# nghiant03/spine-vision

Measured on AMD Instinct MI355X. Metric: images/sec training, ConvNeXt-base 512x512 loc, bs32, at 1/2/4/8 MI355X, higher is better.
Workload: dtype bf16; 1 GPU; CoordinateRegressor(convnext_base) localization train step fwd+bwd+allreduce+clip+AdamW; image_size=512, batch_per_gpu=32, global_batch=32, parallelism=dp1, hip_graph=False

## Files before the change

### include/sv_kernels.h

```cpp
#ifndef SV_KERNELS_H
#define SV_KERNELS_H

#include <stdint.h>

#ifdef __cplusplus
extern "C" {
#endif

typedef struct ihipStream_t* sv_stream_t;

typedef enum { SV_F32 = 0, SV_BF16 = 1 } sv_dtype;

typedef enum {
  SV_OK = 0,
  SV_ERR_INVALID_ARG = 1,
  SV_ERR_UNSUPPORTED = 2,
  SV_ERR_LAUNCH = 3
} sv_status;

int sv_version(void);
const char* sv_last_error_string(void);
const char* sv_build_target(void);

typedef struct sv_ctx sv_ctx;
// ... 372 lines not shown
                   void* out, int32_t out_dtype, int64_t rows, int32_t C, int32_t* ctl, float* ws, sv_stream_t stream);
int sv_bn_bwd_apply_fold(int32_t mode, const void* dout, int32_t dout_dtype, const uint8_t* pool_idx, int32_t pool_H,
                         int32_t pool_W, const void* y, int32_t y_dtype, const float* mean, const float* rstd,
                         const float* gamma, const float* beta, const void* y2, int32_t y2_dtype, const float* mean2,
                         const float* rstd2, const float* gamma2, const float* part, const float* part2,
                         int32_t nparts, void* dx, void* dx2, int32_t dx_dtype, float* dgamma, float* dbeta,
                         float* dgamma2, float* dbeta2, int32_t batch_stats, int64_t rows, int32_t C, int32_t* ctl,
                         float* ws, sv_stream_t stream);
int sv_relu_mask(const void* dout, int32_t dout_dtype, const void* act, int32_t act_dtype, float* g, int64_t n,
                 sv_stream_t stream);
int sv_maxpool3s2_fwd(const void* x, int32_t x_dtype, void* y, uint8_t* idx, int32_t B, int32_t H, int32_t W,
                      int32_t C, sv_stream_t stream);
int sv_maxpool3s2_bwd(const void* dout, int32_t dout_dtype, const uint8_t* idx, void* dx, int32_t dx_dtype,
                      int32_t B, int32_t H, int32_t W, int32_t C, sv_stream_t stream);
int sv_avgpool_fwd(const void* x, int32_t x_dtype, float* feat, int32_t B, int32_t HW, int32_t C,
                   sv_stream_t stream);
int sv_avgpool_bwd(const float* dfeat, void* dx, int32_t dx_dtype, int32_t B, int32_t HW, int32_t C,
                   sv_stream_t stream);

#define SV_HEAD_CE 0
#define SV_HEAD_BCE 1
typedef struct {
  int32_t kind;
  int32_t offset;
  int32_t ncls;
  float weight;
  float label_smoothing;
  const void* target;
  int32_t target_dtype;
} sv_head_task;
int sv_head_loss(const float* logits, int32_t B, int32_t K, const sv_head_task* tasks, int32_t ntasks, float* loss,
                 float* dlogits, sv_stream_t stream);

#ifdef __cplusplus
}
#endif
#endif
```

### spine-vision_amd/kernels.py

```python

from __future__ import annotations

import ctypes
import os

import numpy as np
import torch

from . import native as nv
from .native import SV_BF16, SV_F32, call, dt, ptr, value

EPS_LN = 1e-6


class GemmProbe:

    def __init__(self, key: tuple, name: str = "") -> None:
        self.key = key
        self.name = name
        self.events: list[tuple[torch.cuda.Event, torch.cuda.Event]] = []
        self.flops = 0.0
        self.bytes = 0.0
        self.launches = 0
        self.shares: list[float] = []
# ... 1958 lines not shown
         ptr(rstd), ptr(gamma), ptr(beta), C, ptr(part))
    if (bn_fold_ok(rows, C, P) and rows * C < 2 ** 31
            and _bn_small_args_ok(dpool4d, y2d, mean, rstd, gamma, beta)):
        return _bn_bwd_apply_fold(nv.SV_BN_SMALL_RELU, dpool4d, y2d, mean, rstd, gamma, part, P, idx=idx, H=H, W=W,
                                  beta=beta, dgamma=dgamma, dbeta=dbeta, dx_dtype=dx_dtype, batch_stats=batch_stats,
                                  out=out)
    sums = _bn_bwd_sums(P, C, batch_stats, (part, dgamma, dbeta), sums=sums)
    dx = (torch.empty(rows, C, device=y2d.device, dtype=dx_dtype) if out is None
          else _conv_buf(out, (rows, C), dx_dtype, y2d.device, "bn_relu_bwd_pooled: out"))
    call("sv_bn_relu_bwd_apply_pool", ptr(dpool4d), dt(dpool4d), ptr(idx), B, H, W, ptr(y2d), dt(y2d), ptr(mean),
         ptr(rstd), ptr(gamma), ptr(beta), ptr(sums), ptr(dx), dt(dx), C)
    return dx


def head_loss(logits: torch.Tensor, specs: list) -> tuple:
    _check(logits.dtype == torch.float32 and logits.dim() == 2 and logits.is_contiguous(), "head_loss: logits")
    B, Kc = logits.shape
    cover = 0
    tasks = []
    for kind, off, n, w, sm, t in specs:
        if kind == nv.SV_HEAD_CE:
            _check(t.dtype == torch.int64 and t.is_contiguous() and t.numel() == B, "head_loss: CE target int64 [B]")
        else:
            _check(t.dtype in (torch.float32, torch.bfloat16) and t.is_contiguous() and t.numel() == B * n,
                   "head_loss: BCE target f32 / bf16 [B][ncls]")
        tasks.append(nv.HeadTask(kind, off, n, float(w), float(sm), ptr(t), dt(t) if kind == nv.SV_HEAD_BCE else 0))
        cover += n
    loss = torch.empty((), device=logits.device, dtype=torch.float32)
    dl = (torch.empty_like if cover == Kc else torch.zeros_like)(logits)
    call("sv_head_loss", ptr(logits), B, Kc, (nv.HeadTask * len(tasks))(*tasks), len(tasks), ptr(loss), ptr(dl))
    return loss, dl


def maxpool_fwd(x4d: torch.Tensor, *, out: tuple | None = None):
    B, H, W, C = x4d.shape
    _check(x4d.is_contiguous() and C % 4 == 0, "maxpool_fwd: need contiguous NHWC, C % 4 == 0")
    OH, OW = conv_out_hw(H, W, 3, 2, 1)
    if out is None:
        y = torch.empty(B, OH, OW, C, device=x4d.device, dtype=x4d.dtype)
        idx = torch.empty(B, OH, OW, C, device=x4d.device, dtype=torch.uint8)
    else:
        y = _conv_buf(out[0], (B, OH, OW, C), x4d.dtype, x4d.device, "maxpool_fwd: out")
        idx = _conv_buf(out[1], (B, OH, OW, C), torch.uint8, x4d.device, "maxpool_fwd: out")
    call("sv_maxpool3s2_fwd", ptr(x4d), dt(x4d), ptr(y), ptr(idx), B, H, W, C)
    return y, idx


def maxpool_bwd(dout4d: torch.Tensor, idx: torch.Tensor, H: int, W: int, dx_dtype=torch.float32, *,
                out: torch.Tensor | None = None) -> torch.Tensor:
    B, OH, OW, C = dout4d.shape
    _check(dout4d.is_contiguous() and idx.shape == dout4d.shape and (OH, OW) == conv_out_hw(H, W, 3, 2, 1),
           "maxpool_bwd: shape mismatch")
    dx = (torch.empty(B, H, W, C, device=dout4d.device, dtype=dx_dtype) if out is None
          else _conv_buf(out, (B, H, W, C), dx_dtype, dout4d.device, "maxpool_bwd: out"))
    call("sv_maxpool3s2_bwd", ptr(dout4d), dt(dout4d), ptr(idx), ptr(dx), dt(dx), B, H, W, C)
    return dx


def avgpool_fwd(x4d: torch.Tensor, *, out: torch.Tensor | None = None) -> torch.Tensor:
    B, H, W, C = x4d.shape
    _check(x4d.is_contiguous() and C % 4 == 0, "avgpool_fwd: need contiguous NHWC, C % 4 == 0")
    feat = (torch.empty(B, C, device=x4d.device, dtype=torch.float32) if out is None
            else _conv_buf(out, (B, C), torch.float32, x4d.device, "avgpool_fwd: out"))
    call("sv_avgpool_fwd", ptr(x4d), dt(x4d), ptr(feat), B, H * W, C)
    return feat

# ... 11 lines not shown
```

### spine-vision_amd/native.py

```python

from __future__ import annotations

import ctypes
import os
import re
import threading

import torch

_HERE = os.path.dirname(os.path.abspath(__file__))
LIB_PATH = os.environ.get("SV_LIB_PATH") or os.path.join(_HERE, "libsv_kernels.so")
HEADER = os.path.join(os.path.dirname(_HERE), "include", "sv_kernels.h")

SV_F32, SV_BF16 = 0, 1
SV_IMG_F32_NCHW, SV_IMG_U8_GRAY, SV_IMG_U8_HWC = 0, 1, 2
SV_BN_SMALL_MASK, SV_BN_SMALL_RELU, SV_BN_SMALL_DUAL = 0, 1, 2
SV_HEAD_CE, SV_HEAD_BCE = 0, 1
SV_BN_FOLD_CTL_INTS, SV_BN_FOLD_WS_FLOATS = 256, 2 * 2 * 2048 + 2 * 64 * 16 * 64
(SV_EPI_STORE, SV_EPI_BIAS_GELU2, SV_EPI_BIAS_GAMMA_RES, SV_EPI_GELU_GRAD, SV_EPI_SLAB, SV_EPI_BIAS_GELU_DUAL,
 SV_EPI_MUL_AUX, SV_EPI_BIAS_GELU, SV_EPI_STORE_STATS, SV_EPI_STORE_BN_BWD, SV_EPI_LN_BWD) = range(11)

_p = ctypes.c_void_p
_i32 = ctypes.c_int32
_i64 = ctypes.c_int64
_f32 = ctypes.c_float


class BnRef(ctypes.Structure):
    _fields_ = [("mean", _p), ("rstd", _p), ("gamma", _p), ("beta", _p)]


class GemmPolicy(ctypes.Structure):
    _fields_ = [("impl", _i32), ("grid_cap", _i32), ("wg_per_cu", _i32), ("priority", _i32)]

    def __repr__(self) -> str:
        return (f"GemmPolicy(impl={self.impl}, grid_cap={self.grid_cap}, wg_per_cu={self.wg_per_cu}, "
                f"priority={self.priority})")


class CtxInfo(ctypes.Structure):
    _fields_ = [("device", _i32), ("compute_units", _i32), ("lds_bytes_per_wg", _i32), ("xcds", _i32),
                ("lds_raised_kernels", _i32), ("refs", _i32), ("arch", ctypes.c_char * 32)]


def policy(impl: int = 0, grid_cap: int = 0, wg_per_cu: int = 0, priority: int = 0) -> GemmPolicy:
    return GemmPolicy(int(impl), int(grid_cap or 0), int(wg_per_cu), int(priority))


class GemmDesc(ctypes.Structure):
    _fields_ = [
# ... 149 lines not shown
    "sv_rowscale_add": [_p, _p, _p, _p, _i64, _i64, _i32, _i32, _p],
    "sv_rowscale_cast_bf16": [_p, _p, _p, _i64, _i64, _i32, _i32, _p],
    "sv_patchify16": [_p, _i32, _p, _p, _p, _i32, _i32, _i32, _i32, _i64, _i32, _p],
    "sv_vit_tokens": [_p, _p, _p, _p, _i32, _i32, _i32, _i32, _i32, _p],
    "sv_image_to_nhwc": [_p, _p, _i32, _i32, _i32, _i32, _i32, _i32, _p],
    "sv_image_u8_hwc_to_nhwc": [_p, _p, _p, _p, _i32, _i32, _i32, _i32, _i32, _p],
    "sv_bn_nparts": [_i64, _i32],
    "sv_bn_stats": [_p, _i32, _i64, _i32, _p, _p],
    "sv_bn_stats_finish": [_p, _i32, _p, _i32, _i64, _i32, _f32, _f32, _p, _p, _p, _p, _p, _p, _p, _p],
    "sv_bn_eval_params": [_p, _p, _f32, _p, _p, _i32, _p],
    "sv_bn_act_fwd": [_p, _i32, _p, _p, _p, _p, _p, _i32, _p, _p, _p, _p, _i32, _p, _i32, _i64, _i32, _p],
    "sv_bn_bwd_stats": [_p, _i32, _p, _i32, _p, _i32, _p, _p, _i64, _i32, _p, _p],
    "sv_bn_bwd_stats_mask": [_p, _i32, _p, _i32, _p, _i32, _p, _p, _i64, _i32, _p, _p],
    "sv_bn_bwd_finish": [_p, _i32, _i32, _p, _p, _p, _p, _p, _p],
    "sv_bn_bwd_stats_mask_dual": [_p, _i32, _p, _i32, _p, _i32, _p, _p, _p, _i32, _p, _p, _i64, _i32, _p, _p, _p],
    "sv_bn_bwd_apply_dual": [_p, _i32, _p, _i32, _p, _p, _p, _p, _p, _i32, _p, _p, _p, _p, _p, _p, _i32, _i64, _i32,
                             _p],
    "sv_bn_relu_bwd_stats": [_p, _i32, _p, _i32, _p, _p, _p, _p, _i64, _i32, _p, _p],
    "sv_bn_relu_bwd_apply": [_p, _i32, _p, _i32, _p, _p, _p, _p, _p, _p, _i32, _i64, _i32, _p],
    "sv_bn_relu_bwd_stats_pool": [_p, _i32, _p, _i32, _i32, _i32, _p, _i32, _p, _p, _p, _p, _i32, _p, _p],
    "sv_bn_relu_bwd_apply_pool": [_p, _i32, _p, _i32, _i32, _i32, _p, _i32, _p, _p, _p, _p, _p, _p, _i32, _i32, _p],
    "sv_bn_bwd_apply": [_p, _i32, _p, _i32, _p, _i32, _p, _p, _p, _p, _p, _i32, _p, _i64, _i32, _p],
    "sv_bn_small_ok": [_i64, _i32],
    "sv_bn_bwd_small": [_i32, _p, _i32, _p, _i32, _p, _i32, _p, _p, _p, _p, _p, _i32, _p, _p, _p, _p, _i32, _p, _p,
                        _i32, _p, _p, _p, _p, _i32, _i64, _i32, _p],
    "sv_bn_act_small": [_p, _i32, _p, _i32, _f32, _f32, _p, _p, _p, _p, _p, _p, _p, _p, _i32, _p, _i32, _f32, _f32,
                        _p, _p, _p, _p, _p, _p, _p, _i32, _p, _i32, _i64, _i32, _p],
    "sv_bn_fold_ok": [_i64, _i32, _i32],
    "sv_bn_act_fold": [_p, _i32, _p, _i32, _f32, _f32, _p, _p, _p, _p, _p, _p, _p, _p, _i32, _p, _i32, _f32, _f32,
                       _p, _p, _p, _p, _p, _p, _p, _i32, _p, _i32, _i64, _i32, _p, _p, _p],
    "sv_bn_bwd_apply_fold": [_i32, _p, _i32, _p, _i32, _i32, _p, _i32, _p, _p, _p, _p, _p, _i32, _p, _p, _p, _p, _p,
                             _i32, _p, _p, _i32, _p, _p, _p, _p, _i32, _i64, _i32, _p, _p, _p],
    "sv_head_loss": [_p, _i32, _i32, _p, _i32, _p, _p, _p],
    "sv_relu_mask": [_p, _i32, _p, _i32, _p, _i64, _p],
    "sv_maxpool3s2_fwd": [_p, _i32, _p, _p, _i32, _i32, _i32, _i32, _p],
    "sv_maxpool3s2_bwd": [_p, _i32, _p, _p, _i32, _i32, _i32, _i32, _i32, _p],
    "sv_avgpool_fwd": [_p, _i32, _p, _i32, _i32, _i32, _p],
    "sv_avgpool_bwd": [_p, _p, _i32, _i32, _i32, _i32, _p],
}
_RESTYPES = {"sv_last_error_string": ctypes.c_char_p, "sv_build_target": ctypes.c_char_p,
             "sv_conv_bwd_weight_work_floats": ctypes.c_int64, "sv_gconv_bwd_weight_work_floats": ctypes.c_int64}
_VALUE_FNS = {n for n in _SIGS if n.endswith(("_nparts", "_ws"))} | {"sv_version", "sv_bn_fold_ok", "sv_dwconv7_ln_fused_ok", "sv_conv_bwd_weight_work_floats",
                                                                     "sv_stream_create_cu_reserved", "sv_bn_small_ok",
                                                                     "sv_gconv_bwd_weight_work_floats"}

_NOSTREAM_FNS = {"sv_ctx_create", "sv_ctx_destroy", "sv_ctx_get_info"}

_lib = None
_lock = threading.Lock()


def header_symbols(path: str = HEADER) -> list[str]:
    text = open(path).read()
    text = re.sub(r"/\*.*?\*/", "", text, flags=re.S)
    return sorted(set(re.findall(r"\b(sv_[a-z0-9_]+)\s*\(", text)))


def lib() -> ctypes.CDLL:
    global _lib
    if _lib is not None:
        return _lib
    with _lock:
        if _lib is not None:
            return _lib
        if not os.path.exists(LIB_PATH):
            raise RuntimeError(
                f"spine_vision_amd: native kernel library not found at {LIB_PATH}; "
                "run `python __graft_entry__.py` (hipcc --offload-arch=gfx950) first"
            )
        L = ctypes.CDLL(LIB_PATH)
        missing = [s for s in header_symbols() if not hasattr(L, s)]
        if missing:
            raise RuntimeError(f"spine_vision_amd: {LIB_PATH} lacks symbols {missing}")
        for name, args in _SIGS.items():
            fn = getattr(L, name)
            fn.argtypes = args
# ... 161 lines not shown
```

### spine-vision_amd/training/engine.py

```python

from __future__ import annotations

import os
from collections import deque
from typing import Any, Callable

import torch
import torch.distributed as dist

from .. import kernels as K
from .comm import BufferSync, GradBucketer, broadcast_parameters
from .flat import FlatArena
from .optim import FlatAdamW


class InflightLimiter:

    def __init__(self, max_inflight: int | None = None) -> None:
        if max_inflight is None:
            max_inflight = int(os.environ.get("SV_MAX_INFLIGHT", "2"))
        self.max_inflight = int(max_inflight)
        self._events: deque = deque()

    def step_done(self) -> None:
# ... 214 lines not shown
            static = _clone(inputs)
            torch.cuda.synchronize(self.device)
            graph = torch.cuda.CUDAGraph()
            with torch.cuda.graph(graph):
                self.optimizer.zero_grad()
                loss = fn(self.model, *static)
                loss.backward()
                scale = None
                if self.grad_clip:
                    nc = K.grad_clip_coef(self.arena.grad_flat, self.grad_clip)
                    self.last_grad_norm = nc[0:1]
                    scale = nc[1:2]
                self.optimizer.step_graph(ranges, hyper, grad_scale=scale)
                loss = loss.detach()
            ent = self._graphs[key] = _Graphed(static, graph, loss, hyper, ranges)
        slot = ent.replays % len(ent.ring)
        if ent.ring_events[slot] is not None:
            ent.ring_events[slot].synchronize()
        buf = ent.ring[slot]
        buf.copy_(torch.tensor(vals, dtype=torch.float32))
        ent.hyper.copy_(buf, non_blocking=True)
        ev = torch.cuda.Event()
        ev.record()
        ent.ring_events[slot] = ev
        ent.replays += 1
        _copy_into(ent.static_inputs, inputs)
        ent.graph.replay()
        out = ent.loss.clone()
        if self.limiter is not None:
            self.limiter.step_done()
        return out

    def step_localization(self, image: torch.Tensor, coords: torch.Tensor, mask: torch.Tensor) -> torch.Tensor:
        return self.step_graphed(lambda m, x, c, k: m.get_loss(m(x), c, mask=k), (image, coords, mask))

    def step_classification(self, image: torch.Tensor, targets: dict[str, Any]) -> torch.Tensor:
        return self.step_graphed(lambda m, x, t: m.get_loss(m(x), t), (image, targets))
```

### spine-vision_amd/training/models/generic.py

```python

from __future__ import annotations

import os
from typing import Any, Literal

import numpy as np
import torch
import torch.nn as nn
import torch.nn.functional as F

from ...core.tasks import (
    TaskConfig,
    compute_predictions_for_tasks,
    compute_probabilities_for_tasks,
    create_loss_functions,
    get_strategy,
    get_tasks,
)
from ...native import SV_HEAD_BCE, SV_HEAD_CE
from .backbone import BackboneFactory


class BaseModel(nn.Module):

    @property
    def name(self) -> str:
        raise NotImplementedError

    def predict(self, x: torch.Tensor, **kwargs: Any):
        self.eval()
        with torch.no_grad():
            return self.forward(x, **kwargs)

    def count_parameters(self) -> int:
        return sum(p.numel() for p in self.parameters() if p.requires_grad)

    def freeze_backbone(self) -> None:
        for p in self.backbone.parameters():
            p.requires_grad = False

    def unfreeze_backbone(self) -> None:
        for p in self.backbone.parameters():
            p.requires_grad = True

    def get_features(self, x: torch.Tensor) -> torch.Tensor:
        return self.backbone(x)


_FUSED_HEADS = os.environ.get("SV_FUSED_HEADS", "1") != "0"
_FUSED_LOSS = os.environ.get("SV_FUSED_LOSS", "1") != "0"


class _HeadOutputs(dict):

    logits: torch.Tensor


class _FusedHeadLoss(torch.autograd.Function):

    @staticmethod
    def forward(ctx, logits, specs, *targets):
        from ...kernels import head_loss

        loss, dl = head_loss(logits.detach(), [sp + (t,) for sp, t in zip(specs, targets)])
        ctx.save_for_backward(dl)
        return loss

    @staticmethod
    def backward(ctx, g):
        (dl,) = ctx.saved_tensors
        return (dl * g, None) + (None,) * (len(ctx.needs_input_grad) - 2)


class Classifier(BaseModel):
    def __init__(self, backbone: str = "resnet50", tasks: list[TaskConfig] | None = None, pretrained: bool = True,
                 dropout: float = 0.3, freeze_backbone: bool = False, precision: str | None = None,
                 img_size=None) -> None:
        super().__init__()
        self._backbone_name = backbone
        self._tasks = tasks if tasks is not None else get_tasks()
        self._task_names = [t.name for t in self._tasks]
        self.backbone, self._feature_dim = BackboneFactory.create(backbone, pretrained, precision=precision,
                                                                       img_size=img_size)
        self.dropout = nn.Dropout(dropout)
        self.heads = nn.ModuleDict({t.name: nn.Linear(self._feature_dim, t.num_classes) for t in self._tasks})
        self._loss_functions, self._loss_weights = create_loss_functions(self._tasks)
        if freeze_backbone:
            self.freeze_backbone()

    @property
    def name(self) -> str:
        return f"Classifier-{self._backbone_name}"

    @property
    def task_names(self) -> list[str]:
        return self._task_names

    @property
    def tasks(self) -> list[TaskConfig]:
        return self._tasks

    @property
    def feature_dim(self) -> int:
        return self._feature_dim
# ... 81 lines not shown
        self._num_outputs, self._num_levels = num_outputs, num_levels
        self._loss_type = loss_type
        self.backbone, self._feature_dim = BackboneFactory.create(backbone, pretrained, precision=precision,
                                                                       img_size=img_size)
        self.head = nn.Sequential(
            nn.LayerNorm(self._feature_dim),
            nn.Dropout(dropout),
            nn.Linear(self._feature_dim, 256),
            nn.GELU(),
            nn.Dropout(dropout / 2),
            nn.Linear(256, num_levels * num_outputs),
            nn.Sigmoid(),
        )
        if loss_type not in ("mse", "smooth_l1", "huber"):
            raise ValueError(f"Unknown loss type: {loss_type}")
        if freeze_backbone:
            self.freeze_backbone()

    @property
    def name(self) -> str:
        return f"Regressor-{self._backbone_name}"

    @property
    def feature_dim(self) -> int:
        return self._feature_dim

    @property
    def num_levels(self) -> int:
        return self._num_levels

    def forward(self, x: torch.Tensor, **kwargs: Any) -> torch.Tensor:
        return self.head(self.backbone(x)).view(-1, self._num_levels, self._num_outputs)

    def _elementwise(self, pred: torch.Tensor, target: torch.Tensor) -> torch.Tensor:
        if self._loss_type == "mse":
            return F.mse_loss(pred, target, reduction="none")
        if self._loss_type == "smooth_l1":
            return F.smooth_l1_loss(pred, target, reduction="none", beta=1.0)
        return F.huber_loss(pred, target, reduction="none", delta=0.1)

    def get_loss(self, predictions: torch.Tensor, targets: torch.Tensor, mask: torch.Tensor | None = None,
                 **kwargs: Any) -> torch.Tensor:
        elem = self._elementwise(predictions, targets)
        if mask is None:
            return elem.mean()
        m = (mask != 0).to(elem.dtype).unsqueeze(-1).expand_as(elem)
        return (elem * m).sum() / m.sum().clamp(min=1.0)
```

### spine-vision_amd/training/trainers/localization.py

```python

from __future__ import annotations

from pathlib import Path
from typing import Any, Literal

import numpy as np
import torch

from ..datasets.localization import (
    IDX_TO_LEVEL,
    NUM_LEVELS,
    LocalizationCollator,
    LocalizationDataset,
)
from ..metrics import LocalizationMetrics
from ..models.generic import CoordinateRegressor
from .base import BaseTrainer, TrainingConfig, TrainingResult, logger


class LocalizationConfig(TrainingConfig):
    task: str = "localization"
    backbone: str = "convnext_base"
    pretrained: bool = True
    freeze_backbone_epochs: int = 0
# ... 19 lines not shown
            model = CoordinateRegressor(backbone=config.backbone, num_outputs=2, pretrained=config.pretrained,
                                        dropout=config.dropout, freeze_backbone=config.freeze_backbone_epochs > 0,
                                        num_levels=config.num_levels, loss_type=config.loss_type,
                                        precision=config.effective_precision, img_size=tuple(config.image_size))
        if train_dataset is None:
            train_dataset = LocalizationDataset(Path(config.data_path), split="train", val_ratio=config.val_split,
                                                series_types=config.series_types, sources=config.sources,
                                                image_size=config.image_size, augment=config.augment,
                                                device_transform=config.device_transform,
                                                augment_coords=config.augment_coords)
        if val_dataset is None:
            val_dataset = LocalizationDataset(Path(config.data_path), split="val", val_ratio=config.val_split,
                                              series_types=config.series_types, sources=config.sources,
                                              image_size=config.image_size, augment=False,
                                              device_transform=config.device_transform)
        super().__init__(config, model, train_dataset, val_dataset)
        self.metrics = LocalizationMetrics(pck_thresholds=config.pck_thresholds,
                                           level_names=list(IDX_TO_LEVEL.values()))
        self._backbone_unfrozen = config.freeze_backbone_epochs == 0

    def _collate_fn(self):
        return LocalizationCollator()

    def _unpack_batch(self, batch: dict[str, Any]):
        return batch["image"], batch["coords"]

    def _train_step(self, batch: dict[str, Any]) -> torch.Tensor:
        from ... import kernels as K

        dev = self.device
        image = K.device_images(batch, dev)
        coords = batch["coords"].to(dev, non_blocking=True)
        mask = batch["mask"].to(dev, non_blocking=True)
        return self._optimize(lambda: self.model.get_loss(self.model(image), coords, mask=mask))

    def _validate_epoch(self) -> tuple[float, dict[str, float]]:
        from ... import kernels as K

        self.model.eval()
        total, n = 0.0, 0
        P, T, Mk = [], [], []
        dev = self.device
        with torch.no_grad():
            for batch in self.val_loader:
                coords, mask = (batch[k].to(dev) for k in ("coords", "mask"))
                image = K.device_images(batch, dev) if "resize" in batch else batch["image"].to(dev)
                pred = self.model(image)
                total += float(self.model.get_loss(pred, coords, mask=mask))
                n += 1
                P.append(self._gather(pred).cpu())
                T.append(self._gather(coords).cpu())
                Mk.append(self._gather(mask).cpu())
        if not P:
            return 0.0, {}
        fp, ft, fl = self._flatten_with_mask(torch.cat(P), torch.cat(T), torch.cat(Mk))
        return total / n, self.metrics.compute(fp, ft, fl)

    @staticmethod
    def _flatten_with_mask(predictions, targets, masks):
        sel = masks.numpy() > 0
        lv = np.broadcast_to(np.arange(predictions.shape[1]), sel.shape)
        return predictions.numpy()[sel], targets.numpy()[sel], lv[sel]

    def _compute_metrics(self, predictions, targets) -> dict[str, float]:
        return self.metrics.compute(predictions.numpy(), targets.numpy())

# ... 37 lines not shown
```

Before: 1144 images/sec.

## Fuse localization head LN-MLP-sigmoid-loss into native forward and backward kernels

Adds a native HIP localization head that runs LayerNorm, dropout, FC1, GELU, dropout, FC2, sigmoid and the masked regression loss in two forward kernels, and computes all head gradients in two backward kernels. The trainer and engine call it through a new loss_from_batch path guarded by shape checks. The goal is to replace the many small PyTorch ops and launches in the head and loss with a few fused launches. The head is tiny next to the ConvNeXt-base backbone, so the effect on the whole step is likely small. Dropout masks now come from native_dropout on a cached ones tensor, which changes how randomness is generated.

```diff
diff --git a/include/sv_kernels.h b/include/sv_kernels.h
--- a/include/sv_kernels.h
+++ b/include/sv_kernels.h
@@ -428,6 +428,21 @@
 int sv_head_loss(const float* logits, int32_t B, int32_t K, const sv_head_task* tasks, int32_t ntasks, float* loss,
                  float* dlogits, sv_stream_t stream);
 
+#define SV_LOC_MSE 0
+#define SV_LOC_SMOOTH_L1 1
+#define SV_LOC_HUBER 2
+int sv_loc_head_ok(int32_t F, int32_t H, int32_t O, int32_t L);
+int sv_loc_head_fwd(const float* feat, const float* lnw, const float* lnb, float eps, const float* W1,
+                    const float* b1, const float* W2, const float* b2, const uint8_t* m1, float s1,
+                    const uint8_t* m2, float s2, const float* target, const float* mask, int32_t kind, int32_t B,
+                    int32_t F, int32_t H, int32_t O, int32_t L, float* mean, float* rstd, float* h, float* pred,
+                    float* loss, float* dz, float* dh, float* a, sv_stream_t stream);
+int sv_loc_head_bwd(const float* gout, const float* feat, const float* lnw, const float* lnb, const float* W1,
+                    const uint8_t* m1, float s1, const float* mean, const float* rstd, const float* a,
+                    const float* dz, const float* dh, int32_t B, int32_t F, int32_t H, int32_t O, float* dW1,
+                    float* db1, float* dW2, float* db2, float* dlnw, float* dlnb, float* dxn, float* dfeat,
+                    sv_stream_t stream);
+
 #ifdef __cplusplus
 }
 #endif
diff --git a/spine-vision_amd/csrc/lochead.hip b/spine-vision_amd/csrc/lochead.hip
--- /dev/null
+++ b/spine-vision_amd/csrc/lochead.hip
@@ -0,0 +1,426 @@
+#include <math.h>
+
+#include "common.h"
+
+namespace sv {
+namespace lochead {
+
+constexpr int kH = 256;
+constexpr int kMaxF = 2048;
+constexpr int kKF = kMaxF / 64;
+constexpr int kMaxO = 32;
+constexpr int kRows1 = 4;
+constexpr int kJT = 64;
+constexpr int kRT = 8;
+constexpr int kBC = 32;
+
+__device__ __forceinline__ void gelu_exact(float x, float& g, float& dg) {
+  const float cdf = 0.5f * (1.0f + erff(x * 0.70710678118654752f));
+  const float pdf = 0.3989422804014327f * expf(-0.5f * x * x);
+  g = x * cdf;
+  dg = fmaf(x, pdf, cdf);
+}
+
+__device__ __forceinline__ float ln_drop(float x, float mean, float rstd, float w, float b, float keep) {
+  return fmaf((x - mean) * rstd, w, b) * keep;
+}
+
+__global__ void __launch_bounds__(256) fwd1_kernel(const float* __restrict__ feat, const float* __restrict__ lnw,
+                                                   const float* __restrict__ lnb, float eps,
+                                                   const float* __restrict__ W1, const float* __restrict__ b1,
+                                                   const uint8_t* __restrict__ m1, float s1, int B, int F,
+                                                   float* __restrict__ mean_o, float* __restrict__ rstd_o,
+                                                   float* __restrict__ h) {
+  __shared__ float xs[kRows1][kMaxF];
+  const int lane = threadIdx.x & 63, w = threadIdx.x >> 6;
+  const int KF = F >> 6;
+  const int b = blockIdx.y * kRows1 + w;
+  const int j = blockIdx.x * kRows1 + w;
+  const float* wr = W1 + (size_t)j * F;
+  float wj[kKF];
+#pragma unroll
+  for (int k = 0; k < kKF; ++k) wj[k] = k < KF ? wr[lane + 64 * k] : 0.f;
+  const float bj = b1[j];
+  if (b < B) {
+    const float* xr = feat + (size_t)b * F;
+    float x[kKF], lw[kKF], lb[kKF], keep[kKF];
+#pragma unroll
+    for (int k = 0; k < kKF; ++k) {
+      const int f = lane + 64 * k;
+      x[k] = k < KF ? xr[f] : 0.f;
+      lw[k] = k < KF ? lnw[f] : 0.f;
+      lb[k] = k < KF ? lnb[f] : 0.f;
+      keep[k] = (k < KF && m1) ? (m1[(size_t)b * F + f] ? s1 : 0.f) : 1.f;
+    }
+    float s = 0.f;
+#pragma unroll
+    for (int k = 0; k < kKF; ++k) s += x[k];
+    const float mean = wave_sum(s) / (float)F;
+    float v = 0.f;
+#pragma unroll
+    for (int k = 0; k < kKF; ++k) {
+      const float d = k < KF ? x[k] - mean : 0.f;
+      v = fmaf(d, d, v);
+    }
+    const float rstd = 1.0f / sqrtf(wave_sum(v) / (float)F + eps);
+    if (blockIdx.x == 0 && lane == 0) {
+      mean_o[b] = mean;
+      rstd_o[b] = rstd;
+    }
+#pragma unroll
+    for (int k = 0; k < kKF; ++k)
+      if (k < KF) xs[w][lane + 64 * k] = ln_drop(x[k], mean, rstd, lw[k], lb[k], keep[k]);
+  }
+  __syncthreads();
+#pragma unroll
+  for (int r = 0; r < kRows1; ++r) {
+    const int br = blockIdx.y * kRows1 + r;
+    if (br >= B) break;
+    float acc = 0.f;
+#pragma unroll
+    for (int k = 0; k < kKF; ++k)
+      if (k < KF) acc = fmaf(xs[r][lane + 64 * k], wj[k], acc);
+    acc = wave_sum(acc);
+    if (lane == 0) h[(size_t)br * kH + j] = acc + bj;
+  }
+}
+
+__global__ void __launch_bounds__(1024) fwd2_kernel(const float* __restrict__ h, const float* __restrict__ W2,
+                                                    const float* __restrict__ b2, const uint8_t* __restrict__ m2,
+                                                    float s2, const float* __restrict__ target,
+                                                    const float* __restrict__ mask, int kind, int B, int O, int L,
+                                                    float* __restrict__ pred, float* __restrict__ loss,
+                                                    float* __restrict__ dz, float* __restrict__ dh,
+                                                    float* __restrict__ a_o) {
+  __shared__ float w2s[kMaxO * kH];
+  __shared__ float red[16];
+  const int lane = threadIdx.x & 63, w = threadIdx.x >> 6;
+  const int nout = O / L;
+  float hq[4], kq[4], tq = 0.f, mq = 0.f;
+  auto load_row = [&](int b) {
+#pragma unroll
+    for (int q = 0; q < 4; ++q) {
+      const int k = lane + 64 * q;
+      hq[q] = h[(size_t)b * kH + k];
+      kq[q] = m2 ? (m2[(size_t)b * kH + k] ? s2 : 0.f) : 1.f;
+    }
+    if (lane < O) {
+      tq = target[(size_t)b * O + lane];
+      mq = mask[(size_t)b * L + lane / nout] != 0.f ? 1.f : 0.f;
+    }
+  };
+  if (w < B) load_row(w);
+  const float myb2 = lane < O ? b2[lane] : 0.f;
+  for (int i = threadIdx.x; i < O * kH; i += 1024) w2s[i] = W2[i];
+  float cnt = 0.f;
+  for (int i = threadIdx.x; i < B * L; i += 1024) cnt += mask[i] != 0.f ? 1.f : 0.f;
+  const float den = fmaxf(block_sum(cnt, red) * (float)nout, 1.0f);
+  const float inv_den = 1.0f / den;
+  float lsum = 0.f;
+  for (int b = w; b < B; b += 16) {
+    float a[4], dg[4], keep[4];
+    const float t = tq, mk = mq;
+#pragma unroll
+    for (int q = 0; q < 4; ++q) {
+      float g;
+      gelu_exact(hq[q], g, dg[q]);
+      keep[q] = kq[q];
+      a[q] = g * keep[q];
+    }
+    if (b + 16 < B) load_row(b + 16);
+    float myz = 0.f;
+    for (int o = 0; o < O; ++o) {
+      float p = 0.f;
+#pragma unroll
+      for (int q = 0; q < 4; ++q) p = fmaf(a[q], w2s[o * kH + lane + 64 * q], p);
+      p = wave_sum(p);
+      if (lane == o) myz = p + myb2;
+    }
+    float mydz = 0.f;
+    if (lane < O) {
+      const float pr = 1.0f / (1.0f + expf(-myz));
+      const float d = pr - t, ad = fabsf(d);
+      float elem, gr;
+      if (kind == SV_LOC_MSE) {
+        elem = d * d;
+        gr = 2.0f * d;
+      } else if (kind == SV_LOC_SMOOTH_L1) {
+        elem = ad < 1.0f ? 0.5f * d * d : ad - 0.5f;
+        gr = ad < 1.0f ? d : copysignf(1.0f, d);
+      } else {
+        elem = ad <= 0.1f ? 0.5f * d * d : 0.1f * (ad - 0.05f);
+        gr = ad <= 0.1f ? d : copysignf(0.1f, d);
+      }
+      lsum += elem * mk;
+      mydz = (gr * mk * inv_den) * (pr * (1.0f - pr));
+      pred[(size_t)b * O + lane] = pr;
+      dz[(size_t)b * O + lane] = mydz;
+    }
+    float da[4] = {0.f, 0.f, 0.f, 0.f};
+    for (int o = 0; o < O; ++o) {
+      const float dzo = __shfl(mydz, o);
+#pragma unroll
+      for (int q = 0; q < 4; ++q) da[q] = fmaf(dzo, w2s[o * kH + lane + 64 * q], da[q]);
+    }
+#pragma unroll
+    for (int q = 0; q < 4; ++q) {
+      a_o[(size_t)b * kH + lane + 64 * q] = a[q];
+      dh[(size_t)b * kH + lane + 64 * q] = da[q] * keep[q] * dg[q];
+    }
+  }
+  const float total = block_sum(lsum, red);
+  if (threadIdx.x == 0) loss[0] = total / den;
+}
+
+struct BwdArgs {
+  const float *gout, *feat, *lnw, *lnb, *W1;
+  const uint8_t* m1;
+  float s1;
+  const float *mean, *rstd, *a, *dz, *dh;
+  int B, F, O;
+  float *dW1, *db1, *dW2, *db2, *dlnw, *dlnb, *dxn, *dfeat;
+};
+
+__global__ void __launch_bounds__(256) bwd2_kernel(const BwdArgs p, int nA, int nB) {
+  __shared__ float sm[4096];
+  const int lane = threadIdx.x & 63, w = threadIdx.x >> 6, tid = threadIdx.x;
+  const int B = p.B, F = p.F, O = p.O;
+  const int FT = F >> 6;
+  const float g = p.gout[0];
+  int wg = blockIdx.x;
+  if (wg < nA) {
+    float* dhs = sm;
+    float* xds = sm + 2048;
+    const int f = (wg % FT) * 64 + lane, j0 = (wg / FT) * kJT;
+    const bool first = wg % FT == 0;
+    const float lw = p.lnw[f], lb = p.lnb[f];
+    float acc[16];
+#pragma unroll
+    for (int jj = 0; jj < 16; ++jj) acc[jj] = 0.f;
+    float bsum = 0.f;
+    for (int bc = 0; bc < B; bc += kBC) {
+      float dv[8], xv[8];
+#pragma unroll
+      for (int i = 0; i < 8; ++i) {
+        const int idx = tid + 256 * i, bb = idx >> 6, jj = idx & 63;
+        dv[i] = bc + bb < B ? p.dh[(size_t)(bc + bb) * kH + j0 + jj] : 0.f;
+        const int b = bc + w * 8 + i;
+        if (b < B) {
+          const float keep = p.m1 ? (p.m1[(size_t)b * F + f] ? p.s1 : 0.f) : 1.f;
+          xv[i] = ln_drop(p.feat[(size_t)b * F + f], p.mean[b], p.rstd[b], lw, lb, keep);
+        } else {
+          xv[i] = 0.f;
+        }
+      }
+      __syncthreads();
+#pragma unroll
+      for (int i = 0; i < 8; ++i) {
+        dhs[tid + 256 * i] = dv[i];
+        xds[(w * 8 + i) * 64 + lane] = xv[i];
+      }
+      __syncthreads();
+#pragma unroll 8
+      for (int bb = 0; bb < kBC; ++bb) {
+        const float x = xds[bb * 64 + lane];
+#pragma unroll
+        for (int jj = 0; jj < 16; ++jj) acc[jj] = fmaf(dhs[bb * 64 + w * 16 + jj], x, acc[jj]);
+      }
+      if (first && w == 0)
+        for (int bb = 0; bb < kBC; ++bb) bsum += dhs[bb * 64 + lane];
+    }
+#pragma unroll
+    for (int jj = 0; jj < 16; ++jj) p.dW1[(size_t)(j0 + w * 16 + jj) * F + f] = g * acc[jj];
+    if (first && w == 0) p.db1[j0 + lane] = g * bsum;
+    return;
+  }
+  wg -= nA;
+  if (wg < nB) {
+    float* dhs = sm;
+    float* part = sm + 2048;
+    const int f = (wg % FT) * 64 + lane, b0 = (wg / FT) * kRT;
+#pragma unroll
+    for (int i = 0; i < 8; ++i) {
+      const int idx = tid + 256 * i, r = idx >> 8, j = idx & 255;
+      dhs[idx] = p.dh[(size_t)min(b0 + r, B - 1) * kH + j];
+    }
+    float acc[kRT][4];
+#pragma unroll
+    for (int r = 0; r < kRT; ++r)
+#pragma unroll
+      for (int c = 0; c < 4; ++c) acc[r][c] = 0.f;
+    __syncthreads();
+    for (int jb = 0; jb < 64; jb += 32) {
+      float wv[32];
+#pragma unroll
+      for (int c = 0; c < 32; ++c) wv[c] = p.W1[(size_t)(w * 64 + jb + c) * F + f];
+#pragma unroll
+      for (int c = 0; c < 32; ++c)
+#pragma unroll
+        for (int r = 0; r < kRT; ++r) acc[r][c & 3] = fmaf(dhs[r * kH + w * 64 + jb + c], wv[c], acc[r][c & 3]);
+    }
+#pragma unroll
+    for (int r = 0; r < kRT; ++r)
+      part[(w * kRT + r) * 64 + lane] = (acc[r][0] + acc[r][1]) + (acc[r][2] + acc[r][3]);
+    __syncthreads();
+#pragma unroll
+    for (int rr = 0; rr < 2; ++rr) {
+      const int r = w * 2 + rr, b = b0 + r;
+      if (b < B) {
+        const float s = (part[(0 * kRT + r) * 64 + lane] + part[(1 * kRT + r) * 64 + lane]) +
+                        (part[(2 * kRT + r) * 64 + lane] + part[(3 * kRT + r) * 64 + lane]);
+        const float keep = p.m1 ? (p.m1[(size_t)b * F + f] ? p.s1 : 0.f) : 1.f;
+        p.dxn[(size_t)b * F + f] = g * s * keep;
+      }
+    }
+    return;
+  }
+  {
+    float* dzs = sm;
+    const int cg = wg - nB;
+    const int k = cg * 64 + lane;
+    float acc[kMaxO / 4];
+#pragma unroll
+    for (int i = 0; i < kMaxO / 4; ++i) acc[i] = 0.f;
+    float bsum = 0.f;
+    for (int bc = 0; bc < B; bc += kBC) {
+      float av[kBC];
+#pragma unroll
+      for (int bb = 0; bb < kBC; ++bb) av[bb] = bc + bb < B ? p.a[(size_t)(bc + bb) * kH + k] : 0.f;
+      float zv[4];
+#pragma unroll
+      for (int i = 0; i < 4; ++i) {
+        const int idx = tid + 256 * i, bb = idx >> 5, o = idx & 31;
+        zv[i] = (bc + bb < B && o < O) ? p.dz[(size_t)(bc + bb) * O + o] : 0.f;
+      }
+      __syncthreads();
+#pragma unroll
+      for (int i = 0; i < 4; ++i) dzs[tid + 256 * i] = zv[i];
+      __syncthreads();
+#pragma unroll
+      for (int bb = 0; bb < kBC; ++bb)
+#pragma unroll
+        for (int i = 0; i < kMaxO / 4; ++i)
+          if (w + 4 * i < O) acc[i] = fmaf(dzs[bb * kMaxO + w + 4 * i], av[bb], acc[i]);
+      if (cg == 0 && tid < O)
+        for (int bb = 0; bb < kBC; ++bb) bsum += dzs[bb * kMaxO + tid];
+    }
+#pragma unroll
+    for (int i = 0; i < kMaxO / 4; ++i)
+      if (w + 4 * i < O) p.dW2[(w + 4 * i) * kH + k] = g * acc[i];
+    if (cg == 0 && tid < O) p.db2[tid] = g * bsum;
+  }
+}
+
+__global__ void __launch_bounds__(64) bwd3_kernel(const BwdArgs p) {
+  const int lane = threadIdx.x;
+  const int B = p.B, F = p.F;
+  const int FT = F >> 6;
+  int wg = blockIdx.x;
+  if (wg < FT) {
+    const int f = wg * 64 + lane;
+    float sw = 0.f, sb = 0.f;
+    for (int bc = 0; bc < B; bc += kBC) {
+      float d[kBC], xh[kBC];
+#pragma unroll
+      for (int bb = 0; bb < kBC; ++bb) {
+        const int b = min(bc + bb, B - 1);
+        d[bb] = p.dxn[(size_t)b * F + f];
+        xh[bb] = (p.feat[(size_t)b * F + f] - p.mean[b]) * p.rstd[b];
+      }
+#pragma unroll
+      for (int bb = 0; bb < kBC; ++bb) {
+        if (bc + bb < B) {
+          sw = fmaf(d[bb], xh[bb], sw);
+          sb += d[bb];
+        }
+      }
+    }
+    p.dlnw[f] = sw;
+    p.dlnb[f] = sb;
+    return;
+  }
+  const int b = wg - FT;
+  const float mean = p.mean[b], rstd = p.rstd[b];
+  float gy[kKF], xh[kKF];
+  float s1 = 0.f, s2 = 0.f;
+#pragma unroll
+  for (int k = 0; k < kKF; ++k) {
+    if (k < FT) {
+      const int f = lane + 64 * k;
+      gy[k] = p.dxn[(size_t)b * F + f] * p.lnw[f];
+      xh[k] = (p.feat[(size_t)b * F + f] - mean) * rstd;
+    } else {
+      gy[k] = 0.f;
+      xh[k] = 0.f;
+    }
+  }
+#pragma unroll
+  for (int k = 0; k < kKF; ++k) {
+    s1 += gy[k];
+    s2 = fmaf(gy[k], xh[k], s2);
+  }
+  const float m1 = wave_sum(s1) / (float)F, m2 = wave_sum(s2) / (float)F;
+#pragma unroll
+  for (int k = 0; k < kKF; ++k)
+    if (k < FT) p.dfeat[(size_t)b * F + lane + 64 * k] = rstd * (gy[k] - m1 - xh[k] * m2);
+}
+
+inline bool shape_ok(int B, int F, int H, int O, int L) {
+  return B >= 1 && F >= 64 && F <= kMaxF && F % 64 == 0 && H == kH && O >= 1 && O <= kMaxO && L >= 1 && O % L == 0;
+}
+
+}
+}
+
+using namespace sv;
+
+extern "C" int sv_loc_head_ok(int32_t F, int32_t H, int32_t O, int32_t L) {
+  return lochead::shape_ok(1, F, H, O, L) ? 1 : 0;
+}
+
+extern "C" int sv_loc_head_fwd(const float* feat, const float* lnw, const float* lnb, float eps, const float* W1,
+                               const float* b1, const float* W2, const float* b2, const uint8_t* m1, float s1,
+                               const uint8_t* m2, float s2, const float* target, const float* mask, int32_t kind,
+                               int32_t B, int32_t F, int32_t H, int32_t O, int32_t L, float* mean, float* rstd,
+                               float* h, float* pred, float* loss, float* dz, float* dh, float* a,
+                               sv_stream_t stream) {
+  SV_REQUIRE(feat && lnw && lnb && W1 && b1 && W2 && b2 && target && mask && mean && rstd && h && pred && loss && dz &&
+                 dh && a,
+             "sv_loc_head_fwd: null argument");
+  SV_REQUIRE(kind == SV_LOC_MSE || kind == SV_LOC_SMOOTH_L1 || kind == SV_LOC_HUBER, "sv_loc_head_fwd: bad loss kind %d",
+             (int)kind);
+  SV_REQUIRE(B >= 1 && (long long)B * (F > lochead::kH ? F : lochead::kH) < (1ll << 31), "sv_loc_head_fwd: bad batch %d",
+             (int)B);
+  SV_REQUIRE(eps > 0.f && (!m1 || s1 > 0.f) && (!m2 || s2 > 0.f), "sv_loc_head_fwd: bad eps / dropout scale");
+  if (!lochead::shape_ok(B, F, H, O, L))
+    return set_error(SV_ERR_UNSUPPORTED, "sv_loc_head_fwd: F %d (multiple of 64 up to %d), hidden %d (%d), O %d (<= %d, "
+                     "a multiple of L %d)", (int)F, lochead::kMaxF, (int)H, lochead::kH, (int)O, lochead::kMaxO, (int)L);
+  hipStream_t s = (hipStream_t)stream;
+  const dim3 g1(lochead::kH / lochead::kRows1, (B + lochead::kRows1 - 1) / lochead::kRows1);
+  lochead::fwd1_kernel<<<g1, 256, 0, s>>>(feat, lnw, lnb, eps, W1, b1, m1, s1, B, F, mean, rstd, h);
+  lochead::fwd2_kernel<<<1, 1024, 0, s>>>(h, W2, b2, m2, s2, target, mask, kind, B, O, L, pred, loss, dz, dh, a);
+  return check_launch("sv_loc_head_fwd");
+}
+
+extern "C" int sv_loc_head_bwd(const float* gout, const float* feat, const float* lnw, const float* lnb,
+                               const float* W1, const uint8_t* m1, float s1, const float* mean, const float* rstd,
+                               const float* a, const float* dz, const float* dh, int32_t B, int32_t F, int32_t H,
+                               int32_t O, float* dW1, float* db1, float* dW2, float* db2, float* dlnw, float* dlnb,
+                               float* dxn, float* dfeat, sv_stream_t stream) {
+  SV_REQUIRE(gout && feat && lnw && lnb && W1 && mean && rstd && a && dz && dh && dW1 && db1 && dW2 && db2 && dlnw &&
+                 dlnb && dxn,
+             "sv_loc_head_bwd: null argument (only m1 and dfeat may be null)");
+  SV_REQUIRE(B >= 1 && (long long)B * (F > lochead::kH ? F : lochead::kH) < (1ll << 31), "sv_loc_head_bwd: bad batch %d",
+             (int)B);
+  if (!lochead::shape_ok(B, F, H, O, O))
+    return set_error(SV_ERR_UNSUPPORTED, "sv_loc_head_bwd: F %d (multiple of 64 up to %d), hidden %d (%d), O %d (<= %d)",
+                     (int)F, lochead::kMaxF, (int)H, lochead::kH, (int)O, lochead::kMaxO);
+  hipStream_t s = (hipStream_t)stream;
+  const lochead::BwdArgs args{gout, feat, lnw, lnb, W1, m1, s1, mean, rstd, a, dz, dh, B, F, O,
+                              dW1, db1, dW2, db2, dlnw, dlnb, dxn, dfeat};
+  const int FT = F / 64;
+  const int nA = FT * (lochead::kH / lochead::kJT), nB = FT * ((B + lochead::kRT - 1) / lochead::kRT);
+  lochead::bwd2_kernel<<<nA + nB + lochead::kH / 64, 256, 0, s>>>(args, nA, nB);
+  lochead::bwd3_kernel<<<FT + (dfeat ? B : 0), 64, 0, s>>>(args);
+  return check_launch("sv_loc_head_bwd");
+}
diff --git a/spine-vision_amd/kernels.py b/spine-vision_amd/kernels.py
--- a/spine-vision_amd/kernels.py
+++ b/spine-vision_amd/kernels.py
@@ -2014,6 +2014,80 @@
     return loss, dl
 
 
+LOC_LOSS_KINDS = {"mse": nv.SV_LOC_MSE, "smooth_l1": nv.SV_LOC_SMOOTH_L1, "huber": nv.SV_LOC_HUBER}
+
+
+def loc_head_ok(F: int, H: int, O: int, L: int) -> bool:
+    return bool(value("sv_loc_head_ok", int(F), int(H), int(O), int(L)))
+
+
+def _pad64(n: int) -> int:
+    return (n + 63) // 64 * 64
+
+
+def _loc_f32(t: torch.Tensor, shape: tuple, who: str) -> None:
+    _check(t.dtype == torch.float32 and t.is_contiguous() and tuple(t.shape) == tuple(shape),
+           f"loc_head: {who} must be contiguous float32 {tuple(shape)}, got {tuple(t.shape)} {t.dtype}")
+
+
+def _loc_keep(m: torch.Tensor | None, p: float, shape: tuple, who: str) -> float:
+    if m is None:
+        return 1.0
+    _check(m.dtype == torch.bool and m.is_contiguous() and tuple(m.shape) == tuple(shape),
+           f"loc_head: {who} must be a contiguous torch.bool {tuple(shape)} keep-mask, got {tuple(m.shape)} {m.dtype}")
+    _check(0.0 <= p < 1.0, f"loc_head: dropout probability {p} of {who} outside [0, 1)")
+    return 1.0 / (1.0 - p)
+
+
+def loc_head_fwd(feat: torch.Tensor, lnw: torch.Tensor, lnb: torch.Tensor, eps: float, W1: torch.Tensor,
+                 b1: torch.Tensor, W2: torch.Tensor, b2: torch.Tensor, target: torch.Tensor, mask: torch.Tensor,
+                 kind: str, m1: torch.Tensor | None = None, p1: float = 0.0, m2: torch.Tensor | None = None,
+                 p2: float = 0.0):
+    _check(feat.dim() == 2 and W1.dim() == 2 and W2.dim() == 2 and mask.dim() == 2, "loc_head: feat, W1, W2, mask 2-D")
+    B, F = feat.shape
+    H, O, L = W1.shape[0], W2.shape[0], mask.shape[1]
+    _check(kind in LOC_LOSS_KINDS, f"loc_head: unknown loss {kind!r}")
+    _loc_f32(feat, (B, F), "feat")
+    _loc_f32(lnw, (F,), "LayerNorm weight")
+    _loc_f32(lnb, (F,), "LayerNorm bias")
+    _loc_f32(W1, (H, F), "W1")
+    _loc_f32(b1, (H,), "b1")
+    _loc_f32(W2, (O, H), "W2")
+    _loc_f32(b2, (O,), "b2")
+    _loc_f32(mask, (B, L), "level mask")
+    _check(target.dtype == torch.float32 and target.is_contiguous() and target.numel() == B * O,
+           f"loc_head: targets must be contiguous float32 with {B * O} elements, got {tuple(target.shape)} {target.dtype}")
+    s1 = _loc_keep(m1, p1, (B, F), "m1")
+    s2 = _loc_keep(m2, p2, (B, H), "m2")
+    dev = feat.device
+    stats = torch.empty(2, B, device=dev, dtype=torch.float32)
+    hid = torch.empty(3, B, H, device=dev, dtype=torch.float32)
+    n = _pad64(B * O)
+    out = torch.empty(2 * n + 1, device=dev, dtype=torch.float32)
+    pred, dz, loss = out[:B * O].view(B, O), out[n:n + B * O].view(B, O), out[2 * n:].view(())
+    call("sv_loc_head_fwd", ptr(feat), ptr(lnw), ptr(lnb), float(eps), ptr(W1), ptr(b1), ptr(W2), ptr(b2), ptr(m1), s1,
+         ptr(m2), s2, ptr(target), ptr(mask), LOC_LOSS_KINDS[kind], B, F, H, O, L, ptr(stats[0]), ptr(stats[1]),
+         ptr(hid[0]), ptr(pred), ptr(loss), ptr(dz), ptr(hid[1]), ptr(hid[2]))
+    return pred, loss, (stats, hid, dz, m1, s1)
+
+
+def loc_head_bwd(gout: torch.Tensor, feat: torch.Tensor, lnw: torch.Tensor, lnb: torch.Tensor, W1: torch.Tensor,
+                 W2: torch.Tensor, saved: tuple, need_dfeat: bool = True):
+    stats, hid, dz, m1, s1 = saved
+    B, F = feat.shape
+    H, O = W1.shape[0], W2.shape[0]
+    _check(gout.dtype == torch.float32 and gout.numel() == 1 and gout.is_contiguous(), "loc_head: gout 0-dim float32")
+    dev = feat.device
+    sizes = [H * F, H, O * H, O, F, F, B * F, B * F if need_dfeat else 0]
+    buf = torch.empty(sum(_pad64(n) for n in sizes), device=dev, dtype=torch.float32)
+    dW1, db1, dW2, db2, dlnw, dlnb, dxn, dfeat = (seg[:n] for seg, n in zip(buf.split([_pad64(n) for n in sizes]),
+                                                                           sizes))
+    call("sv_loc_head_bwd", ptr(gout), ptr(feat), ptr(lnw), ptr(lnb), ptr(W1), ptr(m1), s1,
+         ptr(stats[0]), ptr(stats[1]), ptr(hid[2]), ptr(dz), ptr(hid[1]), B, F, H, O, ptr(dW1), ptr(db1), ptr(dW2),
+         ptr(db2), ptr(dlnw), ptr(dlnb), ptr(dxn), ptr(dfeat) if need_dfeat else None)
+    return (dfeat.view(B, F) if need_dfeat else None, dlnw, dlnb, dW1.view(H, F), db1, dW2.view(O, H), db2)
+
+
 def maxpool_fwd(x4d: torch.Tensor, *, out: tuple | None = None):
     B, H, W, C = x4d.shape
     _check(x4d.is_contiguous() and C % 4 == 0, "maxpool_fwd: need contiguous NHWC, C % 4 == 0")
diff --git a/spine-vision_amd/native.py b/spine-vision_amd/native.py
--- a/spine-vision_amd/native.py
+++ b/spine-vision_amd/native.py
@@ -16,6 +16,7 @@
 SV_IMG_F32_NCHW, SV_IMG_U8_GRAY, SV_IMG_U8_HWC = 0, 1, 2
 SV_BN_SMALL_MASK, SV_BN_SMALL_RELU, SV_BN_SMALL_DUAL = 0, 1, 2
 SV_HEAD_CE, SV_HEAD_BCE = 0, 1
+SV_LOC_MSE, SV_LOC_SMOOTH_L1, SV_LOC_HUBER = 0, 1, 2
 SV_BN_FOLD_CTL_INTS, SV_BN_FOLD_WS_FLOATS = 256, 2 * 2 * 2048 + 2 * 64 * 16 * 64
 (SV_EPI_STORE, SV_EPI_BIAS_GELU2, SV_EPI_BIAS_GAMMA_RES, SV_EPI_GELU_GRAD, SV_EPI_SLAB, SV_EPI_BIAS_GELU_DUAL,
  SV_EPI_MUL_AUX, SV_EPI_BIAS_GELU, SV_EPI_STORE_STATS, SV_EPI_STORE_BN_BWD, SV_EPI_LN_BWD) = range(11)
@@ -231,6 +232,11 @@
     "sv_bn_bwd_apply_fold": [_i32, _p, _i32, _p, _i32, _i32, _p, _i32, _p, _p, _p, _p, _p, _i32, _p, _p, _p, _p, _p,
                              _i32, _p, _p, _i32, _p, _p, _p, _p, _i32, _i64, _i32, _p, _p, _p],
     "sv_head_loss": [_p, _i32, _i32, _p, _i32, _p, _p, _p],
+    "sv_loc_head_ok": [_i32, _i32, _i32, _i32],
+    "sv_loc_head_fwd": [_p, _p, _p, _f32, _p, _p, _p, _p, _p, _f32, _p, _f32, _p, _p, _i32, _i32, _i32, _i32, _i32,
+                        _i32, _p, _p, _p, _p, _p, _p, _p, _p, _p],
+    "sv_loc_head_bwd": [_p, _p, _p, _p, _p, _p, _f32, _p, _p, _p, _p, _p, _i32, _i32, _i32, _i32, _p, _p, _p, _p, _p,
+                        _p, _p, _p, _p],
     "sv_relu_mask": [_p, _i32, _p, _i32, _p, _i64, _p],
     "sv_maxpool3s2_fwd": [_p, _i32, _p, _p, _i32, _i32, _i32, _i32, _p],
     "sv_maxpool3s2_bwd": [_p, _i32, _p, _p, _i32, _i32, _i32, _i32, _i32, _p],
@@ -240,7 +246,7 @@
 _RESTYPES = {"sv_last_error_string": ctypes.c_char_p, "sv_build_target": ctypes.c_char_p,
              "sv_conv_bwd_weight_work_floats": ctypes.c_int64, "sv_gconv_bwd_weight_work_floats": ctypes.c_int64}
 _VALUE_FNS = {n for n in _SIGS if n.endswith(("_nparts", "_ws"))} | {"sv_version", "sv_bn_fold_ok", "sv_dwconv7_ln_fused_ok", "sv_conv_bwd_weight_work_floats",
-                                                                     "sv_stream_create_cu_reserved", "sv_bn_small_ok",
+                                                                     "sv_stream_create_cu_reserved", "sv_bn_small_ok", "sv_loc_head_ok",
                                                                      "sv_gconv_bwd_weight_work_floats"}
 
 _NOSTREAM_FNS = {"sv_ctx_create", "sv_ctx_destroy", "sv_ctx_get_info"}
diff --git a/spine-vision_amd/training/engine.py b/spine-vision_amd/training/engine.py
--- a/spine-vision_amd/training/engine.py
+++ b/spine-vision_amd/training/engine.py
@@ -270,6 +270,8 @@
         return out
 
     def step_localization(self, image: torch.Tensor, coords: torch.Tensor, mask: torch.Tensor) -> torch.Tensor:
+        if hasattr(self.model, "loss_from_batch"):
+            return self.step_graphed(lambda m, x, c, k: m.loss_from_batch(x, c, k), (image, coords, mask))
         return self.step_graphed(lambda m, x, c, k: m.get_loss(m(x), c, mask=k), (image, coords, mask))
 
     def step_classification(self, image: torch.Tensor, targets: dict[str, Any]) -> torch.Tensor:
diff --git a/spine-vision_amd/training/models/generic.py b/spine-vision_amd/training/models/generic.py
--- a/spine-vision_amd/training/models/generic.py
+++ b/spine-vision_amd/training/models/generic.py
@@ -49,6 +49,7 @@
 
 _FUSED_HEADS = os.environ.get("SV_FUSED_HEADS", "1") != "0"
 _FUSED_LOSS = os.environ.get("SV_FUSED_LOSS", "1") != "0"
+_NATIVE_LOC_HEAD = os.environ.get("SV_NATIVE_LOC_HEAD", "1") != "0"
 
 
 class _HeadOutputs(dict):
@@ -70,6 +71,32 @@
     def backward(ctx, g):
         (dl,) = ctx.saved_tensors
         return (dl * g, None) + (None,) * (len(ctx.needs_input_grad) - 2)
+
+
+class _LocHeadLoss(torch.autograd.Function):
+
+    @staticmethod
+    def forward(ctx, feat, lnw, lnb, W1, b1, W2, b2, coords, mask, kind, eps, m1, p1, m2, p2):
+        from ...kernels import loc_head_fwd
+
+        feat = feat.detach()
+        pred, loss, saved = loc_head_fwd(feat, lnw.detach(), lnb.detach(), eps, W1.detach(), b1.detach(),
+                                         W2.detach(), b2.detach(), coords, mask, kind, m1, p1, m2, p2)
+        ctx.save_for_backward(feat, lnw, lnb, W1, W2)
+        ctx.saved = saved
+        ctx.mark_non_differentiable(pred)
+        return loss, pred
+
+    @staticmethod
+    def backward(ctx, g, _gpred):
+        from ...kernels import loc_head_bwd
+
+        feat, lnw, lnb, W1, W2 = ctx.saved_tensors
+        need = ctx.needs_input_grad
+        grads = loc_head_bwd(g.to(torch.float32).contiguous(), feat, lnw.detach(), lnb.detach(), W1.detach(),
+                             W2.detach(), ctx.saved, need_dfeat=need[0])
+        ctx.saved = None
+        return tuple(gr if nd else None for gr, nd in zip(grads, need[:7])) + (None,) * 8
 
 
 class Classifier(BaseModel):
@@ -217,6 +244,45 @@
     def forward(self, x: torch.Tensor, **kwargs: Any) -> torch.Tensor:
         return self.head(self.backbone(x)).view(-1, self._num_levels, self._num_outputs)
 
+    def _keep_mask(self, B: int, n: int, p: float, device) -> torch.Tensor:
+        cache = self.__dict__.setdefault("_ones", {})
+        ones = cache.get((B, n, device))
+        if ones is None:
+            ones = cache[(B, n, device)] = torch.ones(B, n, device=device, dtype=torch.float32)
+        return torch.native_dropout(ones, p, True)[1]
+
+    def _native_head_ok(self, feat: torch.Tensor, coords: torch.Tensor, mask: torch.Tensor | None) -> bool:
+        from ...kernels import loc_head_ok
+
+        ln, fc1, fc2 = self.head[0], self.head[2], self.head[5]
+        return (_NATIVE_LOC_HEAD and mask is not None and feat.is_cuda and feat.dtype == torch.float32
+                and feat.dim() == 2 and coords.is_cuda and mask.is_cuda and mask.dim() == 2
+                and mask.shape == (feat.shape[0], self._num_levels)
+                and coords.numel() == feat.shape[0] * fc2.out_features
+                and self.head[1].p < 1 and self.head[4].p < 1
+                and ln.elementwise_affine and ln.bias is not None and fc1.bias is not None and fc2.bias is not None
+                and all(p.dtype == torch.float32 and p.is_cuda for p in self.head.parameters())
+                and loc_head_ok(feat.shape[1], fc1.out_features, fc2.out_features, self._num_levels))
+
+    def loss_from_batch(self, x: torch.Tensor, targets: torch.Tensor, mask: torch.Tensor | None = None) -> torch.Tensor:
+        feat = self.backbone(x)
+        if not self._native_head_ok(feat, targets, mask):
+            pred = self.head(feat).view(-1, self._num_levels, self._num_outputs)
+            return self.get_loss(pred, targets, mask=mask)
+        ln, d1, fc1, d2, fc2 = self.head[0], self.head[1], self.head[2], self.head[4], self.head[5]
+        B = feat.shape[0]
+        m1 = m2 = None
+        if self.training:
+            if d1.p > 0:
+                m1 = self._keep_mask(B, feat.shape[1], d1.p, feat.device)
+            if d2.p > 0:
+                m2 = self._keep_mask(B, fc1.out_features, d2.p, feat.device)
+        tgt = targets.to(torch.float32).contiguous()
+        lvl = mask if mask.dtype == torch.float32 else (mask != 0).to(torch.float32)
+        loss, _ = _LocHeadLoss.apply(feat.contiguous(), ln.weight, ln.bias, fc1.weight, fc1.bias, fc2.weight, fc2.bias,
+                                     tgt, lvl.contiguous(), self._loss_type, ln.eps, m1, d1.p, m2, d2.p)
+        return loss
+
     def _elementwise(self, pred: torch.Tensor, target: torch.Tensor) -> torch.Tensor:
         if self._loss_type == "mse":
             return F.mse_loss(pred, target, reduction="none")
diff --git a/spine-vision_amd/training/trainers/localization.py b/spine-vision_amd/training/trainers/localization.py
--- a/spine-vision_amd/training/trainers/localization.py
+++ b/spine-vision_amd/training/trainers/localization.py
@@ -75,6 +75,8 @@
         image = K.device_images(batch, dev)
         coords = batch["coords"].to(dev, non_blocking=True)
         mask = batch["mask"].to(dev, non_blocking=True)
+        if hasattr(self.model, "loss_from_batch"):
+            return self._optimize(lambda: self.model.loss_from_batch(image, coords, mask))
         return self._optimize(lambda: self.model.get_loss(self.model(image), coords, mask=mask))
 
     def _validate_epoch(self) -> tuple[float, dict[str, float]]:
```

After: 1144 images/sec. No clear change (-0.0%).
